# wtfashwin/fraud-detection

Hardware: AMD Instinct MI355X
Metric: train_rows_per_sec (SMOTE k-NN + logistic fit, post-SMOTE rows/s, whole job); AUC; SHAP values/s (higher is better)
Workload: dtype bf16; 1 GPU; model=StandardScaler+SMOTE(k=5)+LogisticRegression(C=1,sgd), global_batch=8000000, seq_len=30, parallelism=dp1, rows_per_gpu=10000000, post_smote_rows_global=15972800, smote_scope=global

## Files before the change

### fraud_detection_amd/csrc/bindings.cpp

```cpp
#include <hip/hip_runtime.h>
#include <pybind11/pybind11.h>
#include <pybind11/stl.h>

#include <algorithm>
#include <atomic>
#include <chrono>
#include <cstring>
#include <memory>
#include <string>
#include <thread>
#include <vector>

#include "kernels/launchers.h"
#include "serve/shm_ring.h"

namespace py = pybind11;
using u = uintptr_t;

template <typename T>
static T* P(u p) { return reinterpret_cast<T*>(p); }
static hipStream_t S(u s) { return reinterpret_cast<hipStream_t>(s); }

static py::dict device_info(int dev) {
  hipDeviceProp_t prop;
// ... 748 lines not shown
     py::arg("inv32"), py::arg("aff"), py::arg("chl") = 0, py::arg("qhl") = 0, py::arg("tmax") = 0);
  m.def("knn_splits", [](int mq_pad, int mc_pad) { return fdx::knn_splits(mq_pad, mc_pad); });
  m.def("knn_lds_splits", [](int mq_pad, int mc_pad) { return fdx::knn_lds_splits(mq_pad, mc_pad); });
  m.def("knn_topk_lds", [](u Q, int mq_pad, int mq, u C, int mc_pad, int mc, int64_t self_off, int k, u oidx,
                           u oscore, u ws_score, u ws_idx, int nsplit, u s) {
    fdx::launch_knn_topk_lds(P<const float>(Q), mq_pad, mq, P<const float>(C), mc_pad, mc, self_off, k, P<int>(oidx),
                             P<float>(oscore), P<float>(ws_score), P<int>(ws_idx), nsplit, S(s));
  });
  m.def("knn3_splits", [](int mq_pad, int mc_pad) { return fdx::knn3_splits(mq_pad, mc_pad); });
  m.def("knn_split", [](u Xp, int m_pad, int role, u hl, u tmax, u s) {
    fdx::launch_knn_split(P<const float>(Xp), m_pad, role, P<uint4>(hl), P<float>(tmax), S(s));
  });
  m.def("knn_topk3", [](u Q, u Qhl, int mq_pad, int mq, u C, u Chl, u tmax, int mc_pad, int mc, int64_t self_off,
                        int k, u oidx, u oscore, u wss, u wsi, int nsplit, u s) {
    fdx::launch_knn_topk3(P<const float>(Q), P<const void>(Qhl), mq_pad, mq, P<const float>(C), P<const void>(Chl),
                          P<const float>(tmax), mc_pad, mc, self_off, k, P<int>(oidx), P<float>(oscore),
                          P<float>(wss), P<int>(wsi), nsplit, S(s));
  });
  m.def("knn_b3top_splits", [](int mq_pad, int mc_pad) { return fdx::knn_b3top_splits(mq_pad, mc_pad); });
  m.def("knn_b3top", [](u Q, u Qhl, int mq_pad, int mq, u C, u Chl, u tmax, int mc_pad, int mc, int64_t self_off,
                        int k, u oidx, u oscore, u wss, u wsi, u wsm, u fail, int nsplit, u s) {
    fdx::launch_knn_b3top(P<const float>(Q), P<const void>(Qhl), mq_pad, mq, P<const float>(C), P<const void>(Chl),
                          P<const float>(tmax), mc_pad, mc, self_off, k, P<int>(oidx), P<float>(oscore),
                          P<float>(wss), P<int>(wsi), P<float>(wsm), P<int>(fail), nsplit, S(s));
  });
  m.def("knn3r_splits", [](int mq_pad, int mc_pad) { return fdx::knn3r_splits(mq_pad, mc_pad); });
  m.attr("KNN3R_LIST_CAP") = fdx::knn3r_list_cap();
  m.def("knn_topk3r", [](u Q, u Qhl, int mq_pad, int mq, u C, u Chl, u tmax, int mc_pad, int mc, int64_t self_off,
                         int k, u oidx, u oscore, u lists, u counts, int nsplit, u s) {
    fdx::launch_knn_topk3r(P<const float>(Q), P<const void>(Qhl), mq_pad, mq, P<const float>(C), P<const void>(Chl),
                           P<const float>(tmax), mc_pad, mc, self_off, k, P<int>(oidx), P<float>(oscore),
                           P<int>(lists), P<int>(counts), nsplit, S(s));
  });
  m.def("knn_topk", [](u Q, int mq_pad, int mq, u C, int mc_pad, int mc, int64_t self_off, int k, u oidx,
                       u oscore, u ws_score, u ws_idx, int nsplit, u s) {
    fdx::launch_knn_topk(P<const float>(Q), mq_pad, mq, P<const float>(C), mc_pad, mc,
                         self_off, k, P<int>(oidx), P<float>(oscore), P<float>(ws_score), P<int>(ws_idx), nsplit,
                         S(s));
  });
  m.def("smote_parents", [](u C, int64_t m_rows, u aff, u out, u s) {
    fdx::launch_smote_parents(P<const float>(C), m_rows, P<const double>(aff), P<uint16_t>(out), S(s));
  });
  m.def("smote_generate", [](u C, int parents_bf16, u nbr, int mq, int k, int64_t q_off, int64_t n_new,
                             int64_t sample_offset, uint64_t seed, uint64_t counter_base, float label, int out_kind,
                             float out_scale, u aff, u out, u s) {
    fdx::launch_smote_generate(P<const void>(C), parents_bf16, P<const int>(nbr), mq, k, q_off, n_new, sample_offset,
                               seed, counter_base, label, out_kind, out_scale, P<const double>(aff), P<void>(out), S(s));
  });

  m.def("kernelshap", [](u X, int E, int d, u a, float bias, u bg, u cb, int nbg, u Z, int nS, int S_pad, int parts,
                         u A, u Az, int link, u phi, u fx, u f0, u ws, u cnt, u s, u stamps) {
    fdx::launch_kernelshap(P<const float>(X), E, d, P<const float>(a), bias, P<const float>(bg), P<const float>(cb),
                           nbg, P<const uint16_t>(Z), nS, S_pad, parts, P<const float>(A), P<const float>(Az), link,
                           P<float>(phi), P<float>(fx), P<float>(f0), P<float>(ws), P<unsigned>(cnt), S(s),
                           P<unsigned long long>(stamps));
  });
  m.def("kernelshap_paired", [](u X, int E, int d, u a, float bias, u bg, u cb, int nbg, u Z, int Ppad, int parts,
                                u A, u Az, int link, u phi, u fx, u f0, u ws, u cnt, u s) {
    fdx::launch_kernelshap_paired(P<const float>(X), E, d, P<const float>(a), bias, P<const float>(bg),
                                  P<const float>(cb), nbg, P<const uint32_t>(Z), Ppad, parts, P<const float>(A),
                                  P<const float>(Az), link, P<float>(phi), P<float>(fx), P<float>(f0), P<float>(ws),
                                  P<unsigned>(cnt), S(s));
  });
  m.def("kernelshap_linear_resident", [](int S_pad, int parts) { return fdx::kernelshap_linear_resident(S_pad, parts); });
  m.def("treeshap", [](u Xs, int ldx, int E, int d, u feat, u thr, u leaf, int T, int depth, float base, u bw,
                       int bw_ld, int n_bg, float f0, u phi, u fx, u f0o, u s) {
// ... 211 lines not shown
```

### fraud_detection_amd/csrc/kernels/knn.hip

```cpp
#include <cmath>
#include <cstdlib>

#include "common.h"
#include "launchers.h"
#include "scaler_finalize.h"

namespace fdx {
namespace {

constexpr int kThreads = 256;
constexpr int kWaves = 4;
constexpr int kMaxK = 8;
constexpr float kNegBig = -3.0e38f;
constexpr int kQFlush = 4;
constexpr int kQCap = kQFlush - 1 + 16 + 1;

__device__ __forceinline__ bool better(float s, int i, float s2, int i2) {
  return s > s2 || (s == s2 && i < i2);
}

template <int K>
__device__ __forceinline__ void topk_insert(float (&bs)[K], int (&bi)[K], float s, int i) {
  if (!better(s, i, bs[K - 1], bi[K - 1])) return;
  bs[K - 1] = s;
// ... 837 lines not shown
#pragma unroll
  for (int k = 0; k < K; ++k) { bs[k] = kNegBig; bi[k] = 0x7fffffff; }
  if (live) {
    bool over = false;
    const int64_t plane = (int64_t)nsplit * qblocks * kWave;
    float T = kNegBig;
    for (int s = 0; s < nsplit; ++s) {
#pragma unroll
      for (int h = 0; h < 2; ++h) over |= counts[((int64_t)s * qblocks + blk) * kWave + j + 32 * h] > kListCap;
      T = fmaxf(T, __int_as_float(counts[plane + ((int64_t)s * qblocks + blk) * kWave + j]));
    }
    if (!over) {
      for (int s = 0; s < nsplit; ++s) {
#pragma unroll
        for (int h = 0; h < 2; ++h) {
          const int64_t cb = ((int64_t)s * qblocks + blk) * kWave + j + 32 * h;
          const int n = counts[cb];
          const float skip = T - 2.0f * __int_as_float(counts[2 * plane + cb]);
          const int2* li = lists + ((int64_t)s * qblocks + blk) * kListCap * kWave + j + 32 * h;
          for (int e = l; e < n; e += 8) {
            const int2 v = li[(int64_t)e * kWave];
            if (__int_as_float(v.x) < skip) continue;
            topk_insert<K>(bs, bi, exact(v.y), v.y);
          }
        }
      }
    } else {
      for (int ci = l; ci < mc; ci += 8)
        if (ci != self_c) topk_insert<K>(bs, bi, exact(ci), ci);
    }
  }
#pragma unroll
  for (int off = 1; off < 8; off <<= 1) {
    float os[K];
    int oi[K];
#pragma unroll
    for (int k = 0; k < K; ++k) {
      os[k] = __shfl_xor(bs[k], off, kWave);
      oi[k] = __shfl_xor(bi[k], off, kWave);
    }
    float ns[K];
    int ni[K];
    int ia = 0, ib = 0;
#pragma unroll
    for (int k = 0; k < K; ++k) {
      float a = kNegBig, b = kNegBig;
      int ai = 0x7fffffff, bj = 0x7fffffff;
#pragma unroll
      for (int u = 0; u < K; ++u) {
        if (u == ia) { a = bs[u]; ai = bi[u]; }
        if (u == ib) { b = os[u]; bj = oi[u]; }
      }
      const bool ta = !better(b, bj, a, ai);
      ns[k] = ta ? a : b;
      ni[k] = ta ? ai : bj;
      ia += ta ? 1 : 0;
      ib += ta ? 0 : 1;
    }
#pragma unroll
    for (int k = 0; k < K; ++k) { bs[k] = ns[k]; bi[k] = ni[k]; }
  }
  if (live && l == 0) {
#pragma unroll
    for (int k = 0; k < K; ++k) {
      out_idx[(int64_t)q * K + k] = bi[k];
      if (out_score) out_score[(int64_t)q * K + k] = bs[k];
// ... 589 lines not shown
  if (s > 6) s = 6;
  if (s < 1) s = 1;
  return s;
}

void launch_knn_topk3r(const float* Q, const void* Qhl, int mq_pad, int mq, const float* C, const void* Chl,
                       const float* tmax, int mc_pad, int mc, int64_t self_offset, int k, int* out_idx,
                       float* out_score, int* lists, int* counts, int nsplit, hipStream_t stream) {
  int2* lists2 = reinterpret_cast<int2*>(lists);
  if (mq_pad % 32 != 0 || mc_pad % 32 != 0) throw std::runtime_error("knn_topk3r: pads must be x32");
  if (mq > mq_pad || mc > mc_pad || nsplit < 1 || lists == nullptr || counts == nullptr)
    throw std::runtime_error("knn_topk3r: bad shapes or missing list workspaces");
  const dim3 grid(mq_pad / 32, nsplit);
  const uint4* qh = reinterpret_cast<const uint4*>(Qhl);
  const uint4* chl = reinterpret_cast<const uint4*>(Chl);
  const unsigned rblocks = (unsigned)(((int64_t)mq * 8 + 255) / 256);
#define FDX_KNN3R(KK)                                                                                       \
  knn_collect_kernel<KK><<<grid, kWave, 0, stream>>>(Q, qh, chl, tmax, mq, mc_pad, mc, self_offset, lists2, counts); \
  knn_rerank_kernel<KK><<<rblocks, 256, 0, stream>>>(Q, C, mq, mc, mq_pad / 32, nsplit, self_offset, lists2, counts, \
                                                     out_idx, out_score)
  switch (k) {
    case 1: FDX_KNN3R(1); break;
    case 2: FDX_KNN3R(2); break;
    case 3: FDX_KNN3R(3); break;
    case 4: FDX_KNN3R(4); break;
    case 5: FDX_KNN3R(5); break;
    case 6: FDX_KNN3R(6); break;
    case 7: FDX_KNN3R(7); break;
    case 8: FDX_KNN3R(8); break;
    default: throw std::runtime_error("knn_topk3r: k must be in [1, 8]");
  }
#undef FDX_KNN3R
  check_launch("knn_topk3r");
}

int knn_b3top_splits(int mq_pad, int mc_pad) {
  static const int cap = resident_cap(knn_b3top_kernel<>, kWave);
  static const int forced = [] {
    const char* e = std::getenv("FDX_KNN_B3_SPLITS");
    return e != nullptr ? std::atoi(e) : 0;
  }();
  const int qblocks = mq_pad / 32, tiles = mc_pad / 32;
  int s = forced > 0 ? forced : cap / (qblocks > 0 ? qblocks : 1);
  if (s > 32) s = 32;
  if (s > tiles / 8) s = tiles / 8;
  if (s < 1) s = 1;
  return s;
}

void launch_knn_b3top(const float* Q, const void* Qhl, int mq_pad, int mq, const float* C, const void* Chl,
                      const float* tmax, int mc_pad, int mc, int64_t self_offset, int k, int* out_idx,
                      float* out_score, float* ws_s, int* ws_i, float* ws_m, int* fail, int nsplit,
                      hipStream_t stream) {
  if (mq_pad % 32 != 0 || mc_pad % 32 != 0) throw std::runtime_error("knn_b3top: pads must be x32");
  if (mq > mq_pad || mc > mc_pad || nsplit < 1 || nsplit > 32 || ws_s == nullptr || ws_i == nullptr || ws_m == nullptr)
    throw std::runtime_error("knn_b3top: bad shapes or missing [nsplit][mq][8] workspaces");
  if (fail == nullptr) throw std::runtime_error("knn_b3top: missing the [1 + mq] failed-query list");
  if (hipMemsetAsync(fail, 0, sizeof(int), stream) != hipSuccess) throw std::runtime_error("knn_b3top: memset");
  if (k < 1 || k > kTopP) throw std::runtime_error("knn_b3top: k must be in [1, 8]");
  const dim3 grid(mq_pad / 32, nsplit);
  knn_b3top_kernel<><<<grid, kWave, 0, stream>>>(Q, reinterpret_cast<const uint4*>(Qhl),
                                                  reinterpret_cast<const uint4*>(Chl), tmax, mq, mc_pad, mc,
                                                  self_offset, ws_s, ws_i, ws_m);
  int lg = merge_log2(nsplit);
  if (lg < 3) lg = 3;
  const unsigned fb = (unsigned)((((int64_t)mq << lg) + 255) / 256);
// ... 49 lines not shown
```

### fraud_detection_amd/csrc/kernels/launchers.h

```cpp
#pragma once
#include <hip/hip_runtime.h>
#include <stdint.h>
#include <cstdlib>
#include <stdexcept>
#include <string>
#include <vector>

namespace fdx {


inline bool sync_launch_mode() {
  static const int mode = [] {
    const char* v = std::getenv("FDX_SYNC_LAUNCH");
    return (v != nullptr && v[0] != '\0' && v[0] != '0') ? 1 : 0;
  }();
  return mode != 0;
}

inline void check_launch(const char* what) {
  hipError_t e = hipGetLastError();
  if (e == hipSuccess && sync_launch_mode()) e = hipDeviceSynchronize();
  if (e != hipSuccess) {
    throw std::runtime_error(std::string("fdx kernel launch failed [") + what +
                             "]: " + hipGetErrorString(e));
// ... 171 lines not shown
                       const SmoteView* sv, RowHole hole, const SgdPersistArgs& a, hipStream_t stream);
int sgd_persist_blocks(int grid_blocks);

void launch_knn_prep(const float* X, int m, int m_pad, int role, float* out, float* outq,
                     const double* aff, uint16_t* P, hipStream_t stream, void* chl = nullptr, void* qhl = nullptr,
                     float* tmax = nullptr);
struct KnnRawStats {
  int d, nparts;
  double n;
  const double* sums;
  const float* pivot;
  const float* colscale;
  double *mean64, *var64, *scale64;
  float *mean32, *inv32;
  double* aff;
};
void launch_knn_prep_raw(const float* Xraw, int m, int m_pad, float* out, float* outq, uint16_t* P,
                         const KnnRawStats& st, hipStream_t stream, void* chl = nullptr, void* qhl = nullptr,
                         float* tmax = nullptr);
int knn_splits(int mq_pad, int mc_pad);
void launch_knn_split(const float* Xp, int m_pad, int role, uint4* hl, float* tmax, hipStream_t stream);
int knn3_splits(int mq_pad, int mc_pad);
int knn_lds_splits(int mq_pad, int mc_pad);
int knn_b3top_splits(int mq_pad, int mc_pad);
void launch_knn_b3top(const float* Q, const void* Qhl, int mq_pad, int mq, const float* C, const void* Chl,
                      const float* tmax, int mc_pad, int mc, int64_t self_offset, int k, int* out_idx,
                      float* out_score, float* ws_s, int* ws_i, float* ws_m, int* fail, int nsplit,
                      hipStream_t stream);
int knn3r_list_cap();
int knn3r_splits(int mq_pad, int mc_pad);
void launch_knn_topk3r(const float* Q, const void* Qhl, int mq_pad, int mq, const float* C, const void* Chl,
                       const float* tmax, int mc_pad, int mc, int64_t self_offset, int k, int* out_idx,
                       float* out_score, int* lists, int* counts, int nsplit, hipStream_t stream);
void launch_knn_topk_lds(const float* Q, int mq_pad, int mq, const float* C, int mc_pad, int mc,
                         int64_t self_offset, int k, int* out_idx, float* out_score, float* ws_score, int* ws_idx,
                         int nsplit, hipStream_t stream);
void launch_knn_topk3(const float* Q, const void* Qhl, int mq_pad, int mq, const float* C, const void* Chl,
                      const float* tmax, int mc_pad, int mc, int64_t self_offset, int k, int* out_idx,
                      float* out_score, float* ws_score, int* ws_idx, int nsplit, hipStream_t stream);
void launch_knn_topk(const float* Q, int mq_pad, int mq, const float* C,
                     int mc_pad, int mc, int64_t self_offset, int k, int* out_idx,
                     float* out_score, float* ws_score, int* ws_idx, int nsplit, hipStream_t stream);

void launch_smote_parents(const float* C, int64_t m, const double* aff, uint16_t* P, hipStream_t stream);
void launch_smote_generate(const void* C, int parents_bf16, const int* nbr, int mq, int k, int64_t q_offset,
                           int64_t n_new, int64_t sample_offset, uint64_t seed, uint64_t counter_base, float label,
                           int out_kind, float out_scale, const double* aff, void* out, hipStream_t stream);

void launch_auc_compact(const float* scores, const uint8_t* labels, int64_t n, float* pos,
                        unsigned long long* counter, hipStream_t stream);
void launch_sort_chunks(float* pos, int64_t npos_cap, const unsigned long long* counter,
                        int chunk, int nchunks, hipStream_t stream);
size_t auc_radix_workspace_bytes(int64_t n);
void auc_radix_layout(int64_t n, size_t off[8]);
void launch_auc_radix(const float* scores, const uint8_t* labels, int64_t n, void* ws, int64_t* res, double* auc,
                      hipStream_t stream);
int pr_scan_tile();
int pr_tile_scan_threads();
size_t pr_workspace_bytes(int64_t n);
void pr_layout(int64_t n, size_t off[6]);
void launch_pr_curve(const float* scores, const uint8_t* labels, int64_t n, void* ws, uint32_t* tp, uint32_t* fp,
                     float* thr, int64_t* res, double* ap, hipStream_t stream);
void launch_auc_count(const float* scores, const uint8_t* labels, int64_t n, const float* pos,
                      const unsigned long long* counter, int chunk, int nchunks,
                      unsigned long long* out_pairs, hipStream_t stream);
void launch_confusion(const float* scores, const uint8_t* labels, int64_t n, float threshold,
// ... 103 lines not shown
```

### fraud_detection_amd/ops/knn.py

```python
from __future__ import annotations

import os

import numpy as np
import torch

from . import reference as ref
from .layout import DEFAULT_FP8_SCALE, DTYPE_KIND, NCOLS, check_rows, storage_kind
from .native import native, ptr, stream_of


def _pad32(n: int) -> int:
    return max(32, (n + 31) // 32 * 32)


def _padded(X: torch.Tensor, n_pad: int) -> torch.Tensor:
    if X.shape[0] == n_pad and X.is_contiguous():
        return X
    out = torch.zeros((n_pad, NCOLS), device=X.device, dtype=torch.float32)
    out[: X.shape[0]] = X
    return out


KNN_BF16X3_MIN_CANDIDATES = 1 << 13


def knn_engine(mq: int, mc: int, engine: str | None = None) -> str:
    e = engine or os.environ.get("FDX_KNN", "auto")
    if e == "auto":
        return "bf16x3r" if mc >= KNN_BF16X3_MIN_CANDIDATES else "fp32"
    if e not in ("fp32", "fp32lds", "bf16x3", "bf16x3r", "b3top"):
        raise ValueError(f"unknown k-NN engine {e!r}")
    return e


def _check_parents(parents: torch.Tensor | None, C: torch.Tensor, affine: torch.Tensor | None) -> int:
    if parents is None:
        if affine is not None:
            raise ValueError("parents_affine without parents")
        return 0
    if parents.dtype != torch.bfloat16 or tuple(parents.shape) != (C.shape[0], NCOLS) or \
            not parents.is_contiguous() or parents.device != C.device:
        raise ValueError("parents must be a contiguous bf16 [mc, 32] tensor on C's device")
    if affine is not None and (affine.dtype != torch.float64 or affine.numel() < 64 or affine.device != C.device):
        raise ValueError("parents_affine must be ScalerStats.aff (float64 [64]) on C's device")
    return ptr(parents)


def knn_topk(Q: torch.Tensor, C: torch.Tensor, k: int = 5, self_offset: int = -1, want_dist: bool = False,
             nsplit: int | None = None, engine: str | None = None, parents: torch.Tensor | None = None,
             parents_affine: torch.Tensor | None = None, _diag: dict | None = None, raw_stats=None,
             _operands: dict | None = None):
    for t, nm in ((Q, "Q"), (C, "C")):
        if t.dim() != 2 or t.shape[1] != NCOLS or t.dtype != torch.float32:
            raise ValueError(f"{nm} must be fp32 [m, 32]")
    mq, mc = Q.shape[0], C.shape[0]
    if not 1 <= k <= 8:
        raise ValueError("k must be in [1, 8]")
    n_valid = mc - (1 if self_offset >= 0 else 0)
    if n_valid < k:
        raise ValueError(f"need at least k={k} candidates besides self, have {n_valid}")
    if self_offset >= 0 and self_offset + mq > mc:
        raise ValueError("self_offset + mq exceeds the candidate set")
    if raw_stats is not None:
        if not Q.is_cuda or Q.data_ptr() != C.data_ptr() or mq != mc or not Q.is_contiguous() or want_dist \
                or parents_affine is not None or raw_stats.aff is None or self_offset != 0:
            raise ValueError("raw_stats: a device self-search (Q is C, self_offset 0) over contiguous raw rows, "
                             "stats with aff, no parents_affine, no distances")
    if not Q.is_cuda:
        if _check_parents(parents, C, parents_affine):
            parents.copy_(smote_parents(C, parents_affine))
        idx, d2 = ref.knn_topk(Q.numpy(), C.numpy(), k, self_offset)
        idx_t = torch.from_numpy(idx)
        return (idx_t, torch.from_numpy(d2.astype(np.float32))) if want_dist else idx_t
    m = native()
    s = stream_of(Q)
    eng = knn_engine(mq, mc, engine)
    mq_pad, mc_pad = _pad32(mq), _pad32(mc)
    if eng == "fp32lds":
        mq_pad = (mq_pad + 127) // 128 * 128
    Qc, Cc = Q.contiguous(), C.contiguous()
    Qp = torch.empty((mq_pad, NCOLS), device=Q.device, dtype=torch.float32)
    Cp = torch.empty((mc_pad, NCOLS), device=C.device, dtype=torch.float32)
    pp = _check_parents(parents, Cc, parents_affine)
    self_search = Qc.data_ptr() == Cc.data_ptr() and mq == mc and mq_pad == mc_pad
    split_done = False
    if eng in ("bf16x3r", "b3top"):
        Qhl = torch.empty((mq_pad, 64), device=Q.device, dtype=torch.bfloat16)
        Chl = torch.empty((mc_pad, 64), device=C.device, dtype=torch.bfloat16)
        tmax = torch.empty(mc_pad // 32, device=C.device, dtype=torch.float32)
    if self_search:
        fuse = eng in ("bf16x3r", "b3top")
        hl = (ptr(Chl), ptr(Qhl), ptr(tmax)) if fuse else (0, 0, 0)
        if raw_stats is not None:
            st = raw_stats
            f = st.take_pending()
            if f is None:
                f = {"sums": None, "n": 0.0, "pivot": None, "colscale": None, "nparts": 0}
            m.knn_prep_raw(ptr(Cc), mc, mc_pad, ptr(Cp), ptr(Qp), pp, s, st.d, f["nparts"], f["n"], ptr(f["sums"]),
                           ptr(f["pivot"]), ptr(f["colscale"]), ptr(st.mean64), ptr(st.var64), ptr(st.scale64),
                           ptr(st.mean32), ptr(st.inv32), ptr(st.aff), *hl)
        else:
            m.knn_prep(ptr(Cc), mc, mc_pad, 2, ptr(Cp), s, ptr(Qp), ptr(parents_affine), pp, *hl)
        split_done = fuse
    else:
        if raw_stats is not None:
            raise ValueError("raw_stats: the fp32lds engine pads its queries apart from the candidates")
        m.knn_prep(ptr(Cc), mc, mc_pad, 0, ptr(Cp), s, 0, ptr(parents_affine), pp)
        m.knn_prep(ptr(Qc), mq, mq_pad, 1, ptr(Qp), s)
    if _operands is not None:
        _operands.update(Cp=Cp, Qp=Qp)
        if eng in ("bf16x3r", "b3top"):
            _operands.update(Chl=Chl, Qhl=Qhl, tmax=tmax)
    idx = torch.empty((mq, k), device=Q.device, dtype=torch.int32)
    score = torch.empty((mq, k), device=Q.device, dtype=torch.float32) if want_dist else None
    if nsplit is not None:
        ns = max(1, int(nsplit))
    else:
        ns = {"fp32": m.knn_splits, "fp32lds": m.knn_lds_splits, "bf16x3": m.knn3_splits,
              "bf16x3r": m.knn3r_splits, "b3top": m.knn_b3top_splits}[eng](mq_pad, mc_pad)
    ws_s = ws_i = None
    if ns > 1 and eng not in ("bf16x3r", "b3top"):
        ws_s = torch.empty((ns, mq, k), device=Q.device, dtype=torch.float32)
        ws_i = torch.empty((ns, mq, k), device=Q.device, dtype=torch.int32)
    if eng == "fp32":
        m.knn_topk(ptr(Qp), mq_pad, mq, ptr(Cp), mc_pad, mc, int(self_offset), int(k), ptr(idx),
                   ptr(score), ptr(ws_s), ptr(ws_i), ns, s)
    elif eng == "fp32lds":
        m.knn_topk_lds(ptr(Qp), mq_pad, mq, ptr(Cp), mc_pad, mc, int(self_offset), int(k), ptr(idx),
                       ptr(score), ptr(ws_s), ptr(ws_i), ns, s)
    elif not split_done:
        if eng == "bf16x3":
            Qhl = torch.empty((mq_pad, 64), device=Q.device, dtype=torch.bfloat16)
            Chl = torch.empty((mc_pad, 64), device=C.device, dtype=torch.bfloat16)
            tmax = torch.empty(mc_pad // 32, device=C.device, dtype=torch.float32)
        m.knn_split(ptr(Cp), mc_pad, 2 if eng in ("b3top", "bf16x3r") else 0, ptr(Chl), ptr(tmax), s)
        m.knn_split(ptr(Qp), mq_pad, 1, ptr(Qhl), 0, s)
    if eng == "b3top":
        ns = min(ns, 32)
        ws_s = torch.empty((ns, mq, 8), device=Q.device, dtype=torch.float32)
        ws_i = torch.empty((ns, mq, 8), device=Q.device, dtype=torch.int32)
        ws_m = torch.empty((ns, mq, 2), device=Q.device, dtype=torch.float32)
        fail = torch.empty(1 + mq, device=Q.device, dtype=torch.int32)
        m.knn_b3top(ptr(Qp), ptr(Qhl), mq_pad, mq, ptr(Cp), ptr(Chl), ptr(tmax), mc_pad, mc, int(self_offset),
                    int(k), ptr(idx), ptr(score), ptr(ws_s), ptr(ws_i), ptr(ws_m), ptr(fail), ns, s)
        if _diag is not None:
            _diag.update(nsplit=ns, exact_scans=int(fail[0].item()))
    elif eng == "bf16x3r":
        nb = ns * (mq_pad // 32) * 64
        lists = torch.empty(nb * m.KNN3R_LIST_CAP * 2, device=Q.device, dtype=torch.int32)
        counts = torch.empty(3 * nb, device=Q.device, dtype=torch.int32)
        m.knn_topk3r(ptr(Qp), ptr(Qhl), mq_pad, mq, ptr(Cp), ptr(Chl), ptr(tmax), mc_pad, mc, int(self_offset),
                     int(k), ptr(idx), ptr(score), ptr(lists), ptr(counts), ns, s)
        if _diag is not None:
            c = counts[:nb].float()
            _diag.update(nsplit=ns, list_cap=int(m.KNN3R_LIST_CAP), mean=float(c.mean()), max=int(c.max()),
                         p99=float(torch.quantile(c[: min(c.numel(), 1 << 24)], 0.99)),
                         over_cap=int((c > m.KNN3R_LIST_CAP).sum()), counts=counts[:nb].view(ns, mq_pad // 32, 64))
    elif eng == "bf16x3":
        m.knn_topk3(ptr(Qp), ptr(Qhl), mq_pad, mq, ptr(Cp), ptr(Chl), ptr(tmax), mc_pad, mc, int(self_offset),
                    int(k), ptr(idx), ptr(score), ptr(ws_s), ptr(ws_i), ns, s)
    if want_dist:
        if _operands is not None:
            _operands.update(score=score)
        qn = (Q[:, :30].double() ** 2).sum(1, keepdim=True)
        return idx, (qn - 2.0 * score.double()).float()
    return idx


def smote_parents(C: torch.Tensor, affine: torch.Tensor | None = None) -> torch.Tensor:
    if C.dtype != torch.float32 or C.dim() != 2 or C.shape[1] != NCOLS:
        raise ValueError("C must be fp32 [m, 32]")
    C = C.contiguous()
    if not C.is_cuda:
        v = C.numpy().copy()
        if affine is not None:
            a = affine.cpu().numpy()
            v[:, :30] = (v[:, :30] * (1.0 / a[32:62]).astype(np.float32)) + a[:30].astype(np.float32)
        return torch.from_numpy(v).to(torch.bfloat16)
    P = torch.empty((C.shape[0], NCOLS), dtype=torch.bfloat16, device=C.device)
    native().smote_parents(ptr(C), C.shape[0], ptr(affine), ptr(P), stream_of(C))
    return P


def smote_generate(C: torch.Tensor, nbr: torch.Tensor, q_offset: int, n_new: int, out: torch.Tensor,
                   seed: int = 42, counter_base: int = 0, label: float = 1.0,
                   fp8_scale: float = DEFAULT_FP8_SCALE, affine: torch.Tensor | None = None,
                   sample_offset: int = 0) -> torch.Tensor:
    if C.dtype not in (torch.float32, torch.bfloat16) or C.dim() != 2 or C.shape[1] != NCOLS:
        raise ValueError("C must be fp32 or bf16 [m, 32]")
    pb = C.dtype == torch.bfloat16
# ... 42 lines not shown
```

Baseline: 17.74 billion rows/s.

## Add two-pass threshold k-NN engine with sparse exact rerank

Adds a bf16x3t k-NN path. A first MFMA pass computes per-row group maxima and a per-query k-th-best threshold. A second pass keeps only candidates above that threshold minus an error margin, and a sparse rerank computes exact fp32 scores for the survivors. Auto engine selection uses it for mid-sized candidate sets with many queries. The goal is fewer candidates reaching exact rerank than the single-pass collect path produces, at the cost of streaming the candidate tiles twice, plus extra launches and workspace.

```diff
diff --git a/fraud_detection_amd/csrc/bindings.cpp b/fraud_detection_amd/csrc/bindings.cpp
--- a/fraud_detection_amd/csrc/bindings.cpp
+++ b/fraud_detection_amd/csrc/bindings.cpp
@@ -804,6 +804,13 @@
                            P<const float>(tmax), mc_pad, mc, self_off, k, P<int>(oidx), P<float>(oscore),
                            P<int>(lists), P<int>(counts), nsplit, S(s));
   });
+  m.def("knn3t_splits", [](int mq_pad, int mc_pad) { return fdx::knn3t_splits(mq_pad, mc_pad); });
+  m.def("knn_topk3t", [](u Q, u Qhl, int mq_pad, int mq, u C, u Chl, u tmax, int mc_pad, int mc, int64_t self_off,
+                         int k, u oidx, u oscore, u lists, u counts, u gmax, u thr, int nsplit, u s) {
+    fdx::launch_knn_topk3t(P<const float>(Q), P<const void>(Qhl), mq_pad, mq, P<const float>(C), P<const void>(Chl),
+                           P<const float>(tmax), mc_pad, mc, self_off, k, P<int>(oidx), P<float>(oscore),
+                           P<int>(lists), P<int>(counts), P<float>(gmax), P<float>(thr), nsplit, S(s));
+  });
   m.def("knn_topk", [](u Q, int mq_pad, int mq, u C, int mc_pad, int mc, int64_t self_off, int k, u oidx,
                        u oscore, u ws_score, u ws_idx, int nsplit, u s) {
     fdx::launch_knn_topk(P<const float>(Q), mq_pad, mq, P<const float>(C), mc_pad, mc,
diff --git a/fraud_detection_amd/csrc/kernels/knn.hip b/fraud_detection_amd/csrc/kernels/knn.hip
--- a/fraud_detection_amd/csrc/kernels/knn.hip
+++ b/fraud_detection_amd/csrc/kernels/knn.hip
@@ -893,6 +893,339 @@
   }
 #pragma unroll
   for (int off = 1; off < 8; off <<= 1) {
+    float os[K];
+    int oi[K];
+#pragma unroll
+    for (int k = 0; k < K; ++k) {
+      os[k] = __shfl_xor(bs[k], off, kWave);
+      oi[k] = __shfl_xor(bi[k], off, kWave);
+    }
+    float ns[K];
+    int ni[K];
+    int ia = 0, ib = 0;
+#pragma unroll
+    for (int k = 0; k < K; ++k) {
+      float a = kNegBig, b = kNegBig;
+      int ai = 0x7fffffff, bj = 0x7fffffff;
+#pragma unroll
+      for (int u = 0; u < K; ++u) {
+        if (u == ia) { a = bs[u]; ai = bi[u]; }
+        if (u == ib) { b = os[u]; bj = oi[u]; }
+      }
+      const bool ta = !better(b, bj, a, ai);
+      ns[k] = ta ? a : b;
+      ni[k] = ta ? ai : bj;
+      ia += ta ? 1 : 0;
+      ib += ta ? 0 : 1;
+    }
+#pragma unroll
+    for (int k = 0; k < K; ++k) { bs[k] = ns[k]; bi[k] = ni[k]; }
+  }
+  if (live && l == 0) {
+#pragma unroll
+    for (int k = 0; k < K; ++k) {
+      out_idx[(int64_t)q * K + k] = bi[k];
+      if (out_score) out_score[(int64_t)q * K + k] = bs[k];
+    }
+  }
+}
+
+__device__ __forceinline__ float knn_query_norm(const float* __restrict__ Q, int qg, int h) {
+  const float4* p = reinterpret_cast<const float4*>(Q + (int64_t)qg * kCols + 16 * h);
+  float s2 = 0.0f;
+#pragma unroll
+  for (int k = 0; k < 4; ++k) {
+    const float4 v = p[k];
+    s2 = fmaf(v.x, v.x, s2);
+    s2 = fmaf(v.y, v.y, s2);
+    if (h == 0 || k < 3) {
+      s2 = fmaf(v.z, v.z, s2);
+      s2 = fmaf(v.w, v.w, s2);
+    }
+  }
+  s2 += __shfl_xor(s2, 32, kWave);
+  return sqrtf(s2) * 1.0001f;
+}
+
+__device__ __forceinline__ float knn_max(float a, float b) { return __builtin_amdgcn_fmed3f(a, b, __builtin_inff()); }
+
+struct KnnQFrag {
+  bf16x8_t h0, h1, l0, l1;
+};
+
+__device__ __forceinline__ KnnQFrag knn_load_qfrag(const uint4* __restrict__ Qhl, int qg, int h) {
+  const uint4* qr = Qhl + (int64_t)qg * 8;
+  return {__builtin_bit_cast(bf16x8_t, qr[h]), __builtin_bit_cast(bf16x8_t, qr[2 + h]),
+          __builtin_bit_cast(bf16x8_t, qr[4 + h]), __builtin_bit_cast(bf16x8_t, qr[6 + h])};
+}
+
+template <typename F>
+__device__ __forceinline__ void knn_stream_tiles(const KnnQFrag& qa, const KnnQFrag& qb,
+                                                 const uint4* __restrict__ Chl, const float* __restrict__ tmax,
+                                                 int lane, int t_lo, int t_hi, F&& use) {
+  auto fetch = [&](int t, uint4 (&a)[4], float& tmv) {
+    const uint4* p = Chl + (int64_t)t * 256 + lane;
+    a[0] = p[0]; a[1] = p[64]; a[2] = p[128]; a[3] = p[192];
+    tmv = tmax[t];
+  };
+  auto score = [&](const uint4 (&c)[4], f32x16_t& acc0, f32x16_t& acc1) {
+    const bf16x8_t ch0 = __builtin_bit_cast(bf16x8_t, c[0]), ch1 = __builtin_bit_cast(bf16x8_t, c[1]);
+    const bf16x8_t cl0 = __builtin_bit_cast(bf16x8_t, c[2]), cl1 = __builtin_bit_cast(bf16x8_t, c[3]);
+    acc0 = __builtin_amdgcn_mfma_f32_32x32x16_bf16(cl0, qa.h0, acc0, 0, 0, 0);
+    acc1 = __builtin_amdgcn_mfma_f32_32x32x16_bf16(cl0, qb.h0, acc1, 0, 0, 0);
+    acc0 = __builtin_amdgcn_mfma_f32_32x32x16_bf16(cl1, qa.h1, acc0, 0, 0, 0);
+    acc1 = __builtin_amdgcn_mfma_f32_32x32x16_bf16(cl1, qb.h1, acc1, 0, 0, 0);
+    acc0 = __builtin_amdgcn_mfma_f32_32x32x16_bf16(ch0, qa.l0, acc0, 0, 0, 0);
+    acc1 = __builtin_amdgcn_mfma_f32_32x32x16_bf16(ch0, qb.l0, acc1, 0, 0, 0);
+    acc0 = __builtin_amdgcn_mfma_f32_32x32x16_bf16(ch1, qa.l1, acc0, 0, 0, 0);
+    acc1 = __builtin_amdgcn_mfma_f32_32x32x16_bf16(ch1, qb.l1, acc1, 0, 0, 0);
+    acc0 = __builtin_amdgcn_mfma_f32_32x32x16_bf16(ch0, qa.h0, acc0, 0, 0, 0);
+    acc1 = __builtin_amdgcn_mfma_f32_32x32x16_bf16(ch0, qb.h0, acc1, 0, 0, 0);
+    acc0 = __builtin_amdgcn_mfma_f32_32x32x16_bf16(ch1, qa.h1, acc0, 0, 0, 0);
+    acc1 = __builtin_amdgcn_mfma_f32_32x32x16_bf16(ch1, qb.h1, acc1, 0, 0, 0);
+  };
+  if (t_lo >= t_hi) return;
+  const int last = t_hi - 1;
+  uint4 ca[4], cb[4];
+  float tma, tmb;
+  fetch(t_lo, ca, tma);
+  fetch(t_lo + 1 < t_hi ? t_lo + 1 : last, cb, tmb);
+  for (int t = t_lo; t < t_hi; t += 2) {
+    {
+      f32x16_t acc0 = {}, acc1 = {};
+      score(ca, acc0, acc1);
+      const float tm = tma;
+      fetch(t + 2 < t_hi ? t + 2 : last, ca, tma);
+      use(t, acc0, acc1, tm);
+    }
+    {
+      f32x16_t acc0 = {}, acc1 = {};
+      score(cb, acc0, acc1);
+      const float tm = tmb;
+      fetch(t + 3 < t_hi ? t + 3 : last, cb, tmb);
+      if (t + 1 < t_hi) use(t + 1, acc0, acc1, tm);
+    }
+  }
+}
+
+__global__ __launch_bounds__(kWave) void knn_groupmax_kernel(const float* __restrict__ Q,
+                                                             const uint4* __restrict__ Qhl,
+                                                             const uint4* __restrict__ Chl,
+                                                             const float* __restrict__ tmax, int qblocks, int mc_pad,
+                                                             int64_t self_offset, float* __restrict__ gmax) {
+  const int lane = threadIdx.x;
+  const int h = lane >> 5, j = lane & 31;
+  const int b0 = 2 * blockIdx.x;
+  const bool has1 = b0 + 1 < qblocks;
+  const int b1 = has1 ? b0 + 1 : b0;
+  const float qn0 = knn_query_norm(Q, b0 * 32 + j, h), qn1 = knn_query_norm(Q, b1 * 32 + j, h);
+  const KnnQFrag qa = knn_load_qfrag(Qhl, b0 * 32 + j, h), qb = knn_load_qfrag(Qhl, b1 * 32 + j, h);
+  const int ts = self_offset >= 0 ? (int)((self_offset + b0 * 32) >> 5) : -4;
+  const int sr = self_offset >= 0 ? (int)((self_offset + b0 * 32) & 31) + j : -64;
+  const int d1 = b1 - b0;
+  float m0[16], m1[16];
+#pragma unroll
+  for (int r = 0; r < 16; ++r) m0[r] = m1[r] = kNegBig;
+  float tmm = 0.0f;
+  const int all_tiles = mc_pad / 32;
+  const int t_lo = (int)(((int64_t)all_tiles * blockIdx.y) / gridDim.y);
+  const int t_hi = (int)(((int64_t)all_tiles * (blockIdx.y + 1)) / gridDim.y);
+  auto take = [&](float (&m)[16], const f32x16_t& acc, int dt) {
+    if (dt == 0 || dt == 1) {
+      const int rs = sr - 32 * dt;
+#pragma unroll
+      for (int r = 0; r < 16; ++r) m[r] = knn_max(m[r], 4 * h + (r & 3) + 8 * (r >> 2) == rs ? kNegBig : acc[r]);
+    } else {
+#pragma unroll
+      for (int r = 0; r < 16; ++r) m[r] = knn_max(m[r], acc[r]);
+    }
+  };
+  knn_stream_tiles(qa, qb, Chl, tmax, lane, t_lo, t_hi,
+                   [&](int t, const f32x16_t& acc0, const f32x16_t& acc1, float tm) {
+                     tmm = fmaxf(tmm, tm);
+                     take(m0, acc0, t - ts);
+                     take(m1, acc1, t - ts - d1);
+                   });
+  float* o0 = gmax + (int64_t)(blockIdx.y * qblocks + b0) * 17 * kWave + lane;
+#pragma unroll
+  for (int r = 0; r < 16; ++r) o0[r * kWave] = m0[r];
+  o0[16 * kWave] = kMarginScale * fmaf(qn0, tmm, 0.5f * tmm * tmm);
+  if (has1) {
+    float* o1 = o0 + 17 * kWave;
+#pragma unroll
+    for (int r = 0; r < 16; ++r) o1[r * kWave] = m1[r];
+    o1[16 * kWave] = kMarginScale * fmaf(qn1, tmm, 0.5f * tmm * tmm);
+  }
+}
+
+template <int K>
+__global__ __launch_bounds__(kWave) void knn_threshold_kernel(const float* __restrict__ gmax, int nsplit, int mq,
+                                                              float* __restrict__ thr) {
+  const int lane = threadIdx.x;
+  const int qg = blockIdx.x * 32 + (lane & 31);
+  float v[16];
+#pragma unroll
+  for (int r = 0; r < 16; ++r) v[r] = kNegBig;
+  float M = 0.0f;
+  for (int s = 0; s < nsplit; ++s) {
+    const float* g = gmax + (int64_t)(s * gridDim.x + blockIdx.x) * 17 * kWave + lane;
+#pragma unroll
+    for (int r = 0; r < 16; ++r) v[r] = fmaxf(v[r], g[r * kWave]);
+    M = fmaxf(M, g[16 * kWave]);
+  }
+  float bs[K];
+#pragma unroll
+  for (int k = 0; k < K; ++k) bs[k] = kNegBig;
+#pragma unroll
+  for (int r = 0; r < 16; ++r) {
+    float x = v[r];
+#pragma unroll
+    for (int k = 0; k < K; ++k) {
+      const float hi = fmaxf(bs[k], x);
+      x = fminf(bs[k], x);
+      bs[k] = hi;
+    }
+  }
+  float ps[K];
+#pragma unroll
+  for (int k = 0; k < K; ++k) ps[k] = __shfl_xor(bs[k], 32, kWave);
+  int ia = 0, ib = 0;
+  float kth = kNegBig;
+#pragma unroll
+  for (int k = 0; k < K; ++k) {
+    float a = kNegBig, b = kNegBig;
+#pragma unroll
+    for (int u = 0; u < K; ++u) { if (u == ia) a = bs[u]; if (u == ib) b = ps[u]; }
+    const bool ta = a >= b;
+    kth = ta ? a : b;
+    ia += ta ? 1 : 0;
+    ib += ta ? 0 : 1;
+  }
+  if (lane < 32) {
+    thr[qg] = qg < mq ? kth - M : __builtin_inff();
+    thr[(int64_t)gridDim.x * 32 + qg] = M;
+  }
+}
+
+__global__ __launch_bounds__(kWave) void knn_filter_kernel(const float* __restrict__ Q, const uint4* __restrict__ Qhl,
+                                                           const uint4* __restrict__ Chl,
+                                                           const float* __restrict__ tmax,
+                                                           const float* __restrict__ thr, int qblocks, int mc_pad,
+                                                           int mc, int64_t self_offset, int2* __restrict__ lists,
+                                                           int* __restrict__ counts) {
+  const int lane = threadIdx.x;
+  const int h = lane >> 5, j = lane & 31;
+  const int b0 = 2 * blockIdx.x;
+  const bool has1 = b0 + 1 < qblocks;
+  const int b1 = has1 ? b0 + 1 : b0;
+  const int qg0 = b0 * 32 + j, qg1 = b1 * 32 + j;
+  const int64_t self0 = self_offset >= 0 ? self_offset + qg0 : -1, self1 = self_offset >= 0 ? self_offset + qg1 : -1;
+  const float qn0 = knn_query_norm(Q, qg0, h), qn1 = knn_query_norm(Q, qg1, h);
+  const KnnQFrag qa = knn_load_qfrag(Qhl, qg0, h), qb = knn_load_qfrag(Qhl, qg1, h);
+  const int64_t mq_pad = (int64_t)qblocks * 32;
+  const float T0 = thr[qg0], M0 = thr[mq_pad + qg0];
+  const float T1 = has1 ? thr[qg1] : __builtin_inff(), M1 = thr[mq_pad + qg1];
+  int cnt0 = 0, cnt1 = 0;
+  const int64_t lbase0 = (int64_t)(blockIdx.y * qblocks + b0) * kListCap * kWave + lane;
+  const int64_t lbase1 = lbase0 + (int64_t)kListCap * kWave;
+  const int all_tiles = mc_pad / 32;
+  const int t_lo = (int)(((int64_t)all_tiles * blockIdx.y) / gridDim.y);
+  const int t_hi = (int)(((int64_t)all_tiles * (blockIdx.y + 1)) / gridDim.y);
+  auto filter = [&](int t, const f32x16_t& acc, float tm, float qn, float T, int64_t self_c, int64_t lbase, int& cnt) {
+    const float mg = kMarginScale * fmaf(qn, tm, 0.5f * tm * tm);
+    const float cut = T - mg;
+    float m4[4];
+#pragma unroll
+    for (int q = 0; q < 4; ++q)
+      m4[q] = knn_max(knn_max(acc[4 * q], acc[4 * q + 1]), knn_max(acc[4 * q + 2], acc[4 * q + 3]));
+    const float mx = knn_max(knn_max(m4[0], m4[1]), knn_max(m4[2], m4[3]));
+    if (!__any(mx >= cut)) return;
+    const int cbase = t * 32 + 4 * h;
+#pragma unroll
+    for (int q = 0; q < 4; ++q) {
+      if (!__any(m4[q] >= cut)) continue;
+#pragma unroll
+      for (int rr = 0; rr < 4; ++rr) {
+        const int ci = cbase + rr + 8 * q;
+        if (acc[4 * q + rr] >= cut && ci != self_c && ci < mc) {
+          if (cnt < kListCap) lists[lbase + (int64_t)cnt * kWave] = make_int2(__float_as_int(acc[4 * q + rr] - mg), ci);
+          ++cnt;
+        }
+      }
+    }
+  };
+  knn_stream_tiles(qa, qb, Chl, tmax, lane, t_lo, t_hi,
+                   [&](int t, const f32x16_t& acc0, const f32x16_t& acc1, float tm) {
+                     filter(t, acc0, tm, qn0, T0, self0, lbase0, cnt0);
+                     filter(t, acc1, tm, qn1, T1, self1, lbase1, cnt1);
+                   });
+  const int64_t ci0 = (int64_t)(blockIdx.y * qblocks + b0) * kWave + lane;
+  const int64_t plane = (int64_t)qblocks * gridDim.y * kWave;
+  counts[ci0] = cnt0;
+  counts[plane + ci0] = __float_as_int(T0);
+  counts[2 * plane + ci0] = __float_as_int(M0);
+  if (has1) {
+    counts[ci0 + kWave] = cnt1;
+    counts[plane + ci0 + kWave] = __float_as_int(T1);
+    counts[2 * plane + ci0 + kWave] = __float_as_int(M1);
+  }
+}
+
+template <int K>
+__global__ __launch_bounds__(256) void knn_rerank_sparse_kernel(const float* __restrict__ Q,
+                                                                const float* __restrict__ C, int mq, int mc,
+                                                                int qblocks, int nsplit, int64_t self_offset,
+                                                                const int2* __restrict__ lists,
+                                                                const int* __restrict__ counts,
+                                                                int* __restrict__ out_idx,
+                                                                float* __restrict__ out_score) {
+  const int gl = blockIdx.x * 256 + threadIdx.x;
+  const int q = gl >> 5, l = gl & 31;
+  const bool live = q < mq;
+  const int qq = live ? q : 0;
+  const int blk = qq >> 5, j = qq & 31;
+  const int64_t self_c = self_offset >= 0 ? self_offset + qq : -1;
+  const float4* qp = reinterpret_cast<const float4*>(Q + (int64_t)qq * kCols);
+  auto exact = [&](int ci) -> float {
+    const float4* c = reinterpret_cast<const float4*>(C + (int64_t)ci * kCols);
+    float acc = 0.0f;
+#pragma unroll
+    for (int k = 0; k < kCols / 4; ++k) {
+      const float4 v = c[k], w = qp[k];
+      acc = fmaf(w.x, v.x, acc);
+      acc = fmaf(w.y, v.y, acc);
+      acc = fmaf(w.z, v.z, acc);
+      acc = fmaf(w.w, v.w, acc);
+    }
+    return acc;
+  };
+  float bs[K];
+  int bi[K];
+#pragma unroll
+  for (int k = 0; k < K; ++k) { bs[k] = kNegBig; bi[k] = 0x7fffffff; }
+  bool over = false;
+  if (live) {
+    for (int u = l; u < 2 * nsplit; u += 32) {
+      const int64_t lb = (int64_t)(u >> 1) * qblocks + blk;
+      const int lane = j + 32 * (u & 1);
+      const int n = counts[lb * kWave + lane];
+      over |= n > kListCap;
+      const int2* li = lists + lb * kListCap * kWave + lane;
+      for (int e = 0; e < (n < kListCap ? n : kListCap); ++e) {
+        const int ci = li[(int64_t)e * kWave].y;
+        topk_insert<K>(bs, bi, exact(ci), ci);
+      }
+    }
+  }
+  const uint64_t ob = __ballot(over);
+  if (live && ((ob >> (threadIdx.x & 32)) & 0xffffffffull) != 0) {
+#pragma unroll
+    for (int k = 0; k < K; ++k) { bs[k] = kNegBig; bi[k] = 0x7fffffff; }
+    for (int ci = l; ci < mc; ci += 32)
+      if (ci != self_c) topk_insert<K>(bs, bi, exact(ci), ci);
+  }
+#pragma unroll
+  for (int off = 1; off < 32; off <<= 1) {
     float os[K];
     int oi[K];
 #pragma unroll
@@ -1548,6 +1881,52 @@
   }
 #undef FDX_KNN3R
   check_launch("knn_topk3r");
+}
+
+int knn3t_splits(int mq_pad, int mc_pad) {
+  static const int cap = resident_cap(knn_filter_kernel, kWave);
+  const int waves = (mq_pad / 32 + 1) / 2, tiles = mc_pad / 32;
+  int s = cap / (waves > 0 ? waves : 1);
+  if (s > 16) s = 16;
+  if (s > tiles / 8) s = tiles / 8;
+  if (s < 1) s = 1;
+  return s;
+}
+
+void launch_knn_topk3t(const float* Q, const void* Qhl, int mq_pad, int mq, const float* C, const void* Chl,
+                       const float* tmax, int mc_pad, int mc, int64_t self_offset, int k, int* out_idx,
+                       float* out_score, int* lists, int* counts, float* gmax, float* thr, int nsplit,
+                       hipStream_t stream) {
+  int2* lists2 = reinterpret_cast<int2*>(lists);
+  if (mq_pad % 32 != 0 || mc_pad % 32 != 0) throw std::runtime_error("knn_topk3t: pads must be x32");
+  if (mq > mq_pad || mc > mc_pad || nsplit < 1 || lists == nullptr || counts == nullptr || gmax == nullptr ||
+      thr == nullptr)
+    throw std::runtime_error("knn_topk3t: bad shapes or missing workspaces");
+  const int qblocks = mq_pad / 32;
+  const dim3 grid((qblocks + 1) / 2, nsplit);
+  const uint4* qh = reinterpret_cast<const uint4*>(Qhl);
+  const uint4* chl = reinterpret_cast<const uint4*>(Chl);
+  const unsigned rblocks = (unsigned)(((int64_t)mq * 32 + 255) / 256);
+  knn_groupmax_kernel<<<grid, kWave, 0, stream>>>(Q, qh, chl, tmax, qblocks, mc_pad, self_offset, gmax);
+#define FDX_KNN3T(KK)                                                                                       \
+  knn_threshold_kernel<KK><<<qblocks, kWave, 0, stream>>>(gmax, nsplit, mq, thr);                           \
+  knn_filter_kernel<<<grid, kWave, 0, stream>>>(Q, qh, chl, tmax, thr, qblocks, mc_pad, mc, self_offset, lists2, \
+                                                counts);                                                    \
+  knn_rerank_sparse_kernel<KK><<<rblocks, 256, 0, stream>>>(Q, C, mq, mc, qblocks, nsplit, self_offset, lists2,   \
+                                                            counts, out_idx, out_score)
+  switch (k) {
+    case 1: FDX_KNN3T(1); break;
+    case 2: FDX_KNN3T(2); break;
+    case 3: FDX_KNN3T(3); break;
+    case 4: FDX_KNN3T(4); break;
+    case 5: FDX_KNN3T(5); break;
+    case 6: FDX_KNN3T(6); break;
+    case 7: FDX_KNN3T(7); break;
+    case 8: FDX_KNN3T(8); break;
+    default: throw std::runtime_error("knn_topk3t: k must be in [1, 8]");
+  }
+#undef FDX_KNN3T
+  check_launch("knn_topk3t");
 }
 
 int knn_b3top_splits(int mq_pad, int mc_pad) {
diff --git a/fraud_detection_amd/csrc/kernels/launchers.h b/fraud_detection_amd/csrc/kernels/launchers.h
--- a/fraud_detection_amd/csrc/kernels/launchers.h
+++ b/fraud_detection_amd/csrc/kernels/launchers.h
@@ -227,6 +227,11 @@
 void launch_knn_topk3r(const float* Q, const void* Qhl, int mq_pad, int mq, const float* C, const void* Chl,
                        const float* tmax, int mc_pad, int mc, int64_t self_offset, int k, int* out_idx,
                        float* out_score, int* lists, int* counts, int nsplit, hipStream_t stream);
+int knn3t_splits(int mq_pad, int mc_pad);
+void launch_knn_topk3t(const float* Q, const void* Qhl, int mq_pad, int mq, const float* C, const void* Chl,
+                       const float* tmax, int mc_pad, int mc, int64_t self_offset, int k, int* out_idx,
+                       float* out_score, int* lists, int* counts, float* gmax, float* thr, int nsplit,
+                       hipStream_t stream);
 void launch_knn_topk_lds(const float* Q, int mq_pad, int mq, const float* C, int mc_pad, int mc,
                          int64_t self_offset, int k, int* out_idx, float* out_score, float* ws_score, int* ws_idx,
                          int nsplit, hipStream_t stream);
diff --git a/fraud_detection_amd/ops/knn.py b/fraud_detection_amd/ops/knn.py
--- a/fraud_detection_amd/ops/knn.py
+++ b/fraud_detection_amd/ops/knn.py
@@ -23,13 +23,18 @@
 
 
 KNN_BF16X3_MIN_CANDIDATES = 1 << 13
+KNN_TWOPASS_MAX_CANDIDATES = 1 << 14
+KNN_TWOPASS_MIN_QUERIES = 1 << 12
+STREAM_ENGINES = ("bf16x3r", "bf16x3t", "b3top")
 
 
 def knn_engine(mq: int, mc: int, engine: str | None = None) -> str:
     e = engine or os.environ.get("FDX_KNN", "auto")
     if e == "auto":
-        return "bf16x3r" if mc >= KNN_BF16X3_MIN_CANDIDATES else "fp32"
-    if e not in ("fp32", "fp32lds", "bf16x3", "bf16x3r", "b3top"):
+        if mc < KNN_BF16X3_MIN_CANDIDATES:
+            return "fp32"
+        return "bf16x3t" if mc <= KNN_TWOPASS_MAX_CANDIDATES and mq >= KNN_TWOPASS_MIN_QUERIES else "bf16x3r"
+    if e not in ("fp32", "fp32lds", "bf16x3", "bf16x3r", "bf16x3t", "b3top"):
         raise ValueError(f"unknown k-NN engine {e!r}")
     return e
 
@@ -85,12 +90,12 @@
     pp = _check_parents(parents, Cc, parents_affine)
     self_search = Qc.data_ptr() == Cc.data_ptr() and mq == mc and mq_pad == mc_pad
     split_done = False
-    if eng in ("bf16x3r", "b3top"):
+    if eng in STREAM_ENGINES:
         Qhl = torch.empty((mq_pad, 64), device=Q.device, dtype=torch.bfloat16)
         Chl = torch.empty((mc_pad, 64), device=C.device, dtype=torch.bfloat16)
         tmax = torch.empty(mc_pad // 32, device=C.device, dtype=torch.float32)
     if self_search:
-        fuse = eng in ("bf16x3r", "b3top")
+        fuse = eng in STREAM_ENGINES
         hl = (ptr(Chl), ptr(Qhl), ptr(tmax)) if fuse else (0, 0, 0)
         if raw_stats is not None:
             st = raw_stats
@@ -110,7 +115,7 @@
         m.knn_prep(ptr(Qc), mq, mq_pad, 1, ptr(Qp), s)
     if _operands is not None:
         _operands.update(Cp=Cp, Qp=Qp)
-        if eng in ("bf16x3r", "b3top"):
+        if eng in STREAM_ENGINES:
             _operands.update(Chl=Chl, Qhl=Qhl, tmax=tmax)
     idx = torch.empty((mq, k), device=Q.device, dtype=torch.int32)
     score = torch.empty((mq, k), device=Q.device, dtype=torch.float32) if want_dist else None
@@ -118,9 +123,9 @@
         ns = max(1, int(nsplit))
     else:
         ns = {"fp32": m.knn_splits, "fp32lds": m.knn_lds_splits, "bf16x3": m.knn3_splits,
-              "bf16x3r": m.knn3r_splits, "b3top": m.knn_b3top_splits}[eng](mq_pad, mc_pad)
+              "bf16x3r": m.knn3r_splits, "bf16x3t": m.knn3t_splits, "b3top": m.knn_b3top_splits}[eng](mq_pad, mc_pad)
     ws_s = ws_i = None
-    if ns > 1 and eng not in ("bf16x3r", "b3top"):
+    if ns > 1 and eng not in STREAM_ENGINES:
         ws_s = torch.empty((ns, mq, k), device=Q.device, dtype=torch.float32)
         ws_i = torch.empty((ns, mq, k), device=Q.device, dtype=torch.int32)
     if eng == "fp32":
@@ -134,7 +139,7 @@
             Qhl = torch.empty((mq_pad, 64), device=Q.device, dtype=torch.bfloat16)
             Chl = torch.empty((mc_pad, 64), device=C.device, dtype=torch.bfloat16)
             tmax = torch.empty(mc_pad // 32, device=C.device, dtype=torch.float32)
-        m.knn_split(ptr(Cp), mc_pad, 2 if eng in ("b3top", "bf16x3r") else 0, ptr(Chl), ptr(tmax), s)
+        m.knn_split(ptr(Cp), mc_pad, 2 if eng in STREAM_ENGINES else 0, ptr(Chl), ptr(tmax), s)
         m.knn_split(ptr(Qp), mq_pad, 1, ptr(Qhl), 0, s)
     if eng == "b3top":
         ns = min(ns, 32)
@@ -146,17 +151,30 @@
                     int(k), ptr(idx), ptr(score), ptr(ws_s), ptr(ws_i), ptr(ws_m), ptr(fail), ns, s)
         if _diag is not None:
             _diag.update(nsplit=ns, exact_scans=int(fail[0].item()))
-    elif eng == "bf16x3r":
-        nb = ns * (mq_pad // 32) * 64
+    elif eng in ("bf16x3r", "bf16x3t"):
+        qb = mq_pad // 32
+        nb = ns * qb * 64
         lists = torch.empty(nb * m.KNN3R_LIST_CAP * 2, device=Q.device, dtype=torch.int32)
         counts = torch.empty(3 * nb, device=Q.device, dtype=torch.int32)
-        m.knn_topk3r(ptr(Qp), ptr(Qhl), mq_pad, mq, ptr(Cp), ptr(Chl), ptr(tmax), mc_pad, mc, int(self_offset),
-                     int(k), ptr(idx), ptr(score), ptr(lists), ptr(counts), ns, s)
+        if eng == "bf16x3r":
+            m.knn_topk3r(ptr(Qp), ptr(Qhl), mq_pad, mq, ptr(Cp), ptr(Chl), ptr(tmax), mc_pad, mc, int(self_offset),
+                         int(k), ptr(idx), ptr(score), ptr(lists), ptr(counts), ns, s)
+        else:
+            gmax = torch.empty(ns * qb * 17 * 64, device=Q.device, dtype=torch.float32)
+            thr = torch.empty(2 * mq_pad, device=Q.device, dtype=torch.float32)
+            m.knn_topk3t(ptr(Qp), ptr(Qhl), mq_pad, mq, ptr(Cp), ptr(Chl), ptr(tmax), mc_pad, mc, int(self_offset),
+                         int(k), ptr(idx), ptr(score), ptr(lists), ptr(counts), ptr(gmax), ptr(thr), ns, s)
+            if _operands is not None:
+                _operands.update(gmax=gmax.view(ns, qb, 17, 64), thr=thr.view(2, mq_pad),
+                                 lists=lists.view(ns, qb, m.KNN3R_LIST_CAP, 64, 2), counts=counts.view(3, ns, qb, 64))
         if _diag is not None:
-            c = counts[:nb].float()
+            cn = counts[:nb].view(ns, qb, 64)
+            c = cn.float().flatten()
+            over_q = (cn > m.KNN3R_LIST_CAP).view(ns, qb, 2, 32).any(2).any(0).flatten()[:mq]
             _diag.update(nsplit=ns, list_cap=int(m.KNN3R_LIST_CAP), mean=float(c.mean()), max=int(c.max()),
                          p99=float(torch.quantile(c[: min(c.numel(), 1 << 24)], 0.99)),
-                         over_cap=int((c > m.KNN3R_LIST_CAP).sum()), counts=counts[:nb].view(ns, mq_pad // 32, 64))
+                         over_cap=int((c > m.KNN3R_LIST_CAP).sum()), counts=cn,
+                         per_query=float(c.sum()) / mq, exact_scans=int(over_q.sum()), scanned=over_q)
     elif eng == "bf16x3":
         m.knn_topk3(ptr(Qp), ptr(Qhl), mq_pad, mq, ptr(Cp), ptr(Chl), ptr(tmax), mc_pad, mc, int(self_offset),
                     int(k), ptr(idx), ptr(score), ptr(ws_s), ptr(ws_i), ns, s)
```

Result: faster. 18.22 billion rows/s, median of 6 (+2.7%).
